# rageworx/libsrcnn

Hardware: AMD Instinct MI355X
Metric: megapixels/sec SRCNN Y-channel (2x upscale) (higher is better)
Workload: dtype f32

## Files before the change

libsrcnn_amd/build.py:

```python
import os
import subprocess
import sys

HERE = os.path.dirname(os.path.abspath(__file__))
CSRC = os.path.join(HERE, "csrc")
LIBDIR = os.path.join(HERE, "lib")
LIB = os.path.join(LIBDIR, "libsrcnn_amd.so")

SOURCES = ["srcnn_kernels.hip", "srcnn_fused_f16.hip", "srcnn_yuv_planes.hip", "srcnn_yuv_packed.hip", "srcnn_rgb.hip", "srcnn_rgb_window.hip", "srcnn_yuv_window.hip", "srcnn_yuv_packed_window.hip", "srcnn_window.hip", "srcnn_rect_list.hip", "srcnn_rgb_rect_list.hip", "srcnn_rect_list_call.cpp", "srcnn_rgb_rect_list_call.cpp", "srcnn_capi.cpp", "srcnn_frames.cpp", "srcnn_pipeline.cpp", "srcnn_comm.cpp", "dropin.cpp"]
DEPS = SOURCES + ["../../tools/srcnntest.cpp", "../../tools/srcnnyuv.cpp", "srcnn_kernels.h", "srcnn_yuv.h", "srcnn_rgb.h", "srcnn_window.h", "srcnn_frame_rules.h", "srcnn_frame_args.hpp", "srcnn_rect_source.hpp", "srcnn_rect_atlas.hpp", "srcnn_rgb_rect_atlas.hpp", "srcnn_rect_list.h", "srcnn_pixel_io.h", "srcnn_colour_rules.h", "srcnn_window_tile.h", "srcnn_yuv_packed_fields.h", "srcnn_host.hpp", "srcnn_owned.hpp", "srcnn_settings.hpp", "srcnn_watchdog.hpp", "resample_table.hpp", "srcnn_weights.inc",
                  "../../include/srcnn_amd.h", "../../include/srcnn_amd_debug.h", "../../include/srcnn_amd_yuv.h", "../../include/srcnn_amd_yuv_ex.h", "../../include/srcnn_amd_yuv_packed.h", "../../include/srcnn_amd_rgb.h", "../../include/srcnn_amd_rect.h", "../../include/srcnn_amd_rect_list.h", "../../include/srcnn_amd_rgb_rect.h", "../../include/srcnn_amd_rgb_rect_list.h", "../../include/srcnn_amd_yuv_rect.h", "../../include/srcnn_amd_yuv_packed_rect.h",
                  "../../include/libsrcnn_dropin.h", "exports.map"]

FLAGS = ["--offload-arch=gfx950", "-O3", "-ffp-contract=off", "-fPIC", "-std=c++17",
         "-fvisibility=hidden", "-Wall", "-Wno-unused-result", "-Wno-unused-value", "-Wno-ignored-attributes", "-D__HIP_PLATFORM_AMD__"]


EXTRA_FLAGS = {"srcnn_fused_f16.hip": ["-fno-slp-vectorize"] + os.environ.get("SRCNN_FUSED_CFLAGS", "").split()}


def hipcc():
    for c in (os.environ.get("HIPCC"), "/opt/rocm/bin/hipcc", "hipcc"):
        if c and (os.path.isabs(c) and os.path.exists(c) or not os.path.isabs(c)):
            return c
# ... 18 lines not shown
def stale():
    if not all(os.path.exists(p) for p in (LIB, STAMP, os.path.join(LIBDIR, "libsrcnn.so"), os.path.join(LIBDIR, "libsrcnn.a"))):
        return True
    try:
        return open(STAMP).read().strip() != source_digest()
    except OSError:
        return True


def _region(src, start_pat, end_pat):
    import re
    m = re.search(start_pat, src)
    if not m:
        return None
    e = re.search(end_pat, src[m.end():])
    return src[m.start():m.end() + (e.start() if e else len(src) - m.end())]


def kernel_source_sha(name="k_conv12_mfma"):
    import hashlib
    import re
    src = open(os.path.join(CSRC, "srcnn_kernels.hip")).read()
    m = re.search(r"template <[^>]*>\s*__global__[^\n]*void %s\(" % re.escape(name), src)
    if not m and name == "k_conv3_sparse":
        m = re.search(r"// =+\n// conv3, strict, skipping all-zero channel windows", src)
        if m and not re.search(r"__global__[^\n]*void k_conv3_sparse\(", src[m.end():src.find("// ====", src.find("__global__", m.end()))]):
            m = None
    if not m:
        return None
    end = src.find("// ====", src.find("__global__", m.end()) if name == "k_conv3_sparse" else m.end())
    parts = [src[m.start():end if end > 0 else len(src)]]
    extra = []
    if name == "k_conv12_mfma":
        extra = [_region(src, r"constexpr int M_NW\b", r"\n// One tap-step"),
                 _region(src, r"__device__ __forceinline__ void rs_dma_dword\(", r"\n}\n"),
                 _region(src, r"void conv12_grid_info\(", r"\n}\n"),
                 _region(src, r"void launch_conv12_mfma\(", r"\n}\n"),
                 _region(open(os.path.join(CSRC, "srcnn_capi.cpp")).read(), r"void run_conv12\(", r"\n}\n")]
    elif name == "k_conv3":
        extra = [_region(src, r"constexpr int C3_TW\b", r"\ntemplate <bool STRICT"),
                 _region(src, r"__device__ __forceinline__ void rs_dma_dword\(", r"\n}\n"),
                 _region(src, r"void launch_conv3\(", r"\n}\n")]
    elif name == "k_conv3_sparse":
        extra = [_region(src, r"constexpr int C3_TW\b", r"\ntemplate <bool STRICT"),
                 _region(src, r"__device__ __forceinline__ void rs_dma_dword\(", r"\n}\n"),
                 _region(src, r"void launch_layer3\(", r"\n}\n"),
                 _region(src, r"void launch_conv3\(", r"\n}\n")]
    if any(e is None for e in extra):
        return None
    h = hashlib.sha256()
    for part in parts + extra:
        h.update(part.encode())
        h.update(b"\0")
    return h.hexdigest()


STRICT_DIR = os.path.join(LIBDIR, "strict")
STRICT_LIB = os.path.join(STRICT_DIR, "libsrcnn_amd.so")


def build_strict_only(force=False, verbose=True):
# ... 76 lines not shown
```

libsrcnn_amd/csrc/srcnn_capi.cpp:

```cpp
#include <dlfcn.h>
#include <hip/hip_runtime.h>
#include <sys/prctl.h>
#include <sys/syscall.h>
#include <unistd.h>

#include <algorithm>
#include <cstdio>
#include <cstdlib>
#include <cstring>
#include <string>
#include <thread>

#include "resample_table.hpp"
#include <chrono>
#include <sys/auxv.h>
#include <unistd.h>

#include "../../include/srcnn_amd_rect.h"
#include "srcnn_frame_args.hpp"
#include "srcnn_host.hpp"
#include "srcnn_rect_source.hpp"
#include "srcnn_window.h"

namespace srcnn {
// ... 674 lines not shown
{
    unsigned long long* clk = nullptr;
    if (G.clock_probe.load(std::memory_order_relaxed) && c.cx->clock_buf)
        clk = c.cx->clock_buf + 2 * (size_t)(c.cx->clock_n.fetch_add(1) % kClockSlots);
    unsigned* queue = nullptr;
    hipStreamCaptureStatus cap = hipStreamCaptureStatusNone;
    const bool foreign_capture = c.s && c.ws && !c.ws->frozen && hipStreamIsCapturing(c.s, &cap) == hipSuccess && cap == hipStreamCaptureStatusActive;
    if (foreign_capture) clk = nullptr;
    if (c.ws && settings().conv12_queue && !foreign_capture) {
        if (c.ws->queue && c.ws->queue_dirty) {
            if (hipMemsetAsync(c.ws->queue, 0, 2 * sizeof(unsigned), c.s) == hipSuccess) c.ws->queue_dirty = false;
            else (void)hipGetLastError();
        }
        if (!c.ws->queue && !c.ws->frozen) {
            void* q = nullptr;
            if (hipMalloc(&q, 2 * sizeof(unsigned)) == hipSuccess && hipMemsetAsync(q, 0, 2 * sizeof(unsigned), c.s) == hipSuccess) c.ws->queue = static_cast<unsigned*>(q);
            else { (void)hipFree(q); (void)hipGetLastError(); }
        }
        queue = c.ws->queue;
    }
    launch_conv12_mfma(Y, W, H, y_row_base, y_rows, C2, plane, row0, rows, c.relax(), c.cx->num_cus, c.s, clk, queue);
}

DevAxisTable view_of(const TableRef& t) { return t->view(); }

int resample_src_rows(Call& c, const YSource& src, unsigned sw, unsigned sh, unsigned dw, unsigned dh, int filter,
                      unsigned r0, unsigned r1, float* d_dst)
{
    Workspace& ws = *c.ws;
    hipStream_t s = c.s;
    const float* d_in = src.plane;
    if (sw == dw && sh == dh) {
        if (!d_in) return fail(SRCNN_E_UNSUPPORTED, "identity-size resample needs a float plane");
        HIP_TRY(hipMemcpyAsync(d_dst, d_in + (size_t)r0 * sw, sizeof(float) * (size_t)(r1 - r0) * sw,
                               hipMemcpyDeviceToDevice, s));
        return SRCNN_OK;
    }
    TableRef tv, th;
    int rc;
    if (dw > sw && sh != dh) {
        if ((rc = get_table(c, filter, dw, sw, th))) return rc;
        if ((rc = get_table(c, filter, dh, sh, tv))) return rc;
        if (!settings().resample_2pass &&
            launch_rs2d(src, sw, sh, d_dst, dw, dh, r0, r1 - r0, view_of(tv), view_of(th), s)) return SRCNN_OK;
    }
    if (!d_in) return fail(SRCNN_E_UNSUPPORTED, "this resample shape needs a float source plane");
// ... 107 lines not shown
    if (fused) {
        {
            StageTimer t(SRCNN_STAGE_RESAMPLE, c);
            if ((rc = resample_src_rows(c, src, w, h, dw, dh, filter, ua, ub, ws.up.data()))) return rc;
        }
        {
            StageTimer t(SRCNN_STAGE_CONV12, c);
            launch_fused_f16(ws.up.data(), (int)dw, (int)dh, (int)ua, (int)(ub - ua), d_out, (int)r0, (int)(r1 - r0), cx.fused_w.data(),
                             cx.num_cus, c.s);
        }
        HIP_TRY(hipGetLastError());
        return SRCNN_OK;
    }
#endif
    if ((rc = ws.grow(ws.c2, (size_t)C2N * dw * (cb - ca)))) return rc;
    TraceRange tr("srcnn y_path rows [%u,%u) of %ux%u", r0, r1, dw, dh);
    {
        StageTimer t(SRCNN_STAGE_RESAMPLE, c);
        if ((rc = resample_src_rows(c, src, w, h, dw, dh, filter, ua, ub, ws.up.data()))) return rc;
    }
    const size_t plane = (size_t)dw * (cb - ca);
    {
        StageTimer t(SRCNN_STAGE_CONV12, c);
        run_conv12(c, ws.up.data(), (int)dw, (int)dh, (int)ua, (int)(ub - ua), ws.c2.data(), plane, (int)ca, (int)(cb - ca));
    }
    {
        StageTimer t(SRCNN_STAGE_CONV3, c);
        launch_layer3(ws.c2.data(), plane, (int)dw, (int)dh, (int)ca, (int)(cb - ca), d_out, (int)r0, (int)(r1 - r0),
                     c.relax(), c.s);
    }
    if (const hipError_t e = hipGetLastError(); e != hipSuccess) {
        ws.queue_dirty = true;
        return fail(SRCNN_E_HIP, "y_path_rows: %s", hipGetErrorString(e));
    }
    return SRCNN_OK;
}

int y_path_source_rows(Call& c, unsigned h, unsigned dh, int filter, unsigned r0, unsigned r1, unsigned& lo, unsigned& hi)
{
    const unsigned ca = r0 >= 2 ? r0 - 2 : 0, cb = std::min(dh, r1 + 2);
    const unsigned ua = ca >= 4 ? ca - 4 : 0, ub = std::min(dh, cb + 4);
    if (h == dh) { lo = ua; hi = ub; return SRCNN_OK; }
    TableRef tv;
    int rc = get_table(c, filter, dh, h, tv);
    if (rc) return rc;
    tv->source_span(ua, ub, lo, hi);
    hi = std::min(hi, h);
// ... 85 lines not shown
        {
            StageTimer t(SRCNN_STAGE_RESAMPLE, c);
            if ((rc = resample_window(c, d_in, in_stride, in_x0, in_y0, w, h, dw, dh, filter, uax, ubx, ua, ub, ws.up.data()))) return rc;
        }
        {
            StageTimer t(SRCNN_STAGE_CONV12, c);
            launch_fused_f16(ws.up.data(), (int)Ww, (int)dh, (int)ua, (int)(ub - ua), ws.win.data(), (int)r0, (int)(r1 - r0), cx.fused_w.data(),
                             cx.num_cus, c.s);
        }
        launch_window_copy(interior, Ww, d_out, out_stride, (int)(x1 - x0), (int)(r1 - r0), c.s);
        HIP_TRY(hipGetLastError());
        return SRCNN_OK;
    }
#endif
    if ((rc = ws.grow(ws.c2, (size_t)C2N * Ww * (cb - ca)))) return rc;
    TraceRange tr("srcnn y_path rect [%u,%u)x[%u,%u) of %ux%u", x0, x1, r0, r1, dw, dh);
    {
        StageTimer t(SRCNN_STAGE_RESAMPLE, c);
        if ((rc = resample_window(c, d_in, in_stride, in_x0, in_y0, w, h, dw, dh, filter, uax, ubx, ua, ub, ws.up.data()))) return rc;
    }
    const size_t plane = (size_t)Ww * (cb - ca);
    {
        StageTimer t(SRCNN_STAGE_CONV12, c);
        run_conv12(c, ws.up.data(), (int)Ww, (int)dh, (int)ua, (int)(ub - ua), ws.c2.data(), plane, (int)ca, (int)(cb - ca));
    }
    {
        StageTimer t(SRCNN_STAGE_CONV3, c);
        launch_layer3(ws.c2.data(), plane, (int)Ww, (int)dh, (int)ca, (int)(cb - ca), ws.win.data(), (int)r0, (int)(r1 - r0), c.relax(), c.s);
    }
    launch_window_copy(interior, Ww, d_out, out_stride, (int)(x1 - x0), (int)(r1 - r0), c.s);
    if (const hipError_t e = hipGetLastError(); e != hipSuccess) {
        ws.queue_dirty = true;
        return fail(SRCNN_E_HIP, "y_path_rect: %s", hipGetErrorString(e));
    }
    return SRCNN_OK;
}

}

int y_path_rect(Call& c, const float* d_in, size_t in_stride, unsigned in_x0, unsigned in_y0, unsigned w, unsigned h, unsigned dw,
                unsigned dh, int filter, unsigned x0, unsigned y0, unsigned x1, unsigned y1, float* d_out, size_t out_stride, bool whole_plane)
{
    if (x1 > dw || x0 >= x1 || y1 > dh || y0 >= y1) return fail(SRCNN_E_ARG, "rect [%u,%u)x[%u,%u) outside %ux%u", x0, x1, y0, y1, dw, dh);
    if (dh > (1u << 20) || h > (1u << 20) || dw > 0x7fffffu || (y1 - y0) > 65535u * 16u)
        return fail(SRCNN_E_UNSUPPORTED, "output %ux%u too large", dw, dh);
    if (x0 == 0 && x1 == dw && whole_plane && in_x0 == 0 && in_y0 == 0 && in_stride == w && out_stride == dw)
        return y_path_range(c, d_in, w, h, dw, dh, filter, y0, y1, d_out);
// ... 421 lines not shown

extern "C++" {
namespace srcnn {

int check_rect_geometry(unsigned w, unsigned h, unsigned dw, unsigned dh, int filter, unsigned x0, unsigned y0, unsigned rw, unsigned rh)
{
    if (w == 0 || h == 0 || rw == 0 || rh == 0) return fail(SRCNN_E_ARG, "zero dimension (%ux%u, rect %ux%u)", w, h, rw, rh);
    if (dw == 0 || dh == 0) return fail(SRCNN_E_SCALE, "scaled size %ux%u", dw, dh);
    if (filter < 0 || filter > 4) return fail(SRCNN_E_ARG, "bad filter %d", filter);
    if ((unsigned long long)x0 + rw > dw || (unsigned long long)y0 + rh > dh)
        return fail(SRCNN_E_ARG, "rect %ux%u at (%u,%u) is not inside the %ux%u output", rw, rh, x0, y0, dw, dh);
    return SRCNN_OK;
}

int check_rect_limits(unsigned w, unsigned h, unsigned dw, unsigned dh, unsigned rh)
{
    if (h > (1u << 20) || dh > (1u << 20) || dw > 0x7fffffu || rh > 65535u * 16u || (unsigned long long)w * h > 0x7fffffffULL)
        return fail(SRCNN_E_UNSUPPORTED, "%ux%u -> %ux%u is beyond the Y path's limits", w, h, dw, dh);
    return SRCNN_OK;
}

void run_layers12(const Call& c, const float* Y, int W, int H, int y_row_base, int y_rows, float* C2, size_t plane, int row0, int rows)
{
    run_conv12(c, Y, W, H, y_row_base, y_rows, C2, plane, row0, rows);
}

}
}

int srcnn_rect_abi_version(void) { return SRCNN_AMD_RECT_VERSION; }

int srcnn_y_path_rect_source(unsigned w, unsigned h, unsigned dw, unsigned dh, int filter, unsigned x0, unsigned y0, unsigned rw,
                             unsigned rh, unsigned* sx0, unsigned* sy0, unsigned* sw, unsigned* sh)
{
    int rc;
    if ((rc = check_rect_geometry(w, h, dw, dh, filter, x0, y0, rw, rh))) return rc;
    if ((rc = check_rect_limits(w, h, dw, dh, rh))) return rc;
    unsigned lx, hx, ly, hy;
    y_path_rect_source_span(w, h, dw, dh, filter, x0, y0, x0 + rw, y0 + rh, lx, hx, ly, hy);
    if (sx0) *sx0 = lx;
    if (sy0) *sy0 = ly;
    if (sw) *sw = hx - lx;
    if (sh) *sh = hy - ly;
    return SRCNN_OK;
}

int srcnn_y_path_rect_f32_dev(const float* d_in, size_t in_pitch, unsigned w, unsigned h, unsigned dw, unsigned dh, int filter,
// ... 135 lines not shown

int srcnn_conv3_f32_dev(const float* d_c2, unsigned w, unsigned h, float* d_out, void* stream)
{
    int rc;
    if ((rc = check_plane(d_c2, w, h, d_out))) return rc;
    if (h > 65535u * 16u) return fail(SRCNN_E_UNSUPPORTED, "too many rows");
    if (!ctx_for_stream(stream)) return SRCNN_E_NODEVICE;
    Call c;
    c.mode = G.mode.load();
    launch_layer3(d_c2, (size_t)w * h, (int)w, (int)h, 0, (int)h, d_out, 0, (int)h, c.relax(), (hipStream_t)stream);
    HIP_TRY(hipGetLastError());
    return SRCNN_OK;
}

int srcnn_conv12_f32_dev(const float* d_y, unsigned w, unsigned h, float* d_c2, void* stream)
{
    int rc;
    if ((rc = check_plane(d_y, w, h, d_c2))) return rc;
    if (h > 65535u * 4u) return fail(SRCNN_E_UNSUPPORTED, "too many rows");
    Call c;
    c.cx = ctx_for_stream(stream);
    if (!c.cx) return SRCNN_E_NODEVICE;
    c.s = (hipStream_t)stream; c.mode = G.mode.load();
    run_conv12(c, d_y, (int)w, (int)h, 0, (int)h, d_c2, (size_t)w * h, 0, (int)h);
    HIP_TRY(hipGetLastError());
    return SRCNN_OK;
}

int srcnn_axis_table(int filter, unsigned dst_len, unsigned src_len, int* left, int* right, double* weights)
{
    if (dst_len == 0 || src_len == 0) return fail(SRCNN_E_ARG, "zero length");
    const srcnn::AxisTable t = srcnn::build_axis_table(filter, dst_len, src_len);
    if (left) memcpy(left, t.first.data(), sizeof(int) * dst_len);
    if (right) memcpy(right, t.last.data(), sizeof(int) * dst_len);
    if (weights) memcpy(weights, t.weight.data(), sizeof(double) * t.weight.size());
    return t.window;
}

int srcnn_fused_diag(const float* d_up, unsigned w, unsigned h, float* d_out, unsigned long long* d_dbg, void* stream)
{
    int rc;
    if ((rc = check_plane(d_up, w, h, d_out))) return rc;
#ifdef SRCNN_STRICT_ONLY
    (void)d_dbg; (void)stream;
    return fail(SRCNN_E_UNSUPPORTED, "strict-only build: the fused fp16 kernel is not compiled in");
#else
    Ctx* cx = ctx_for_stream(stream);
// ... 30 lines not shown
```

libsrcnn_amd/csrc/srcnn_kernels.h:

```cpp
#pragma once
#include <hip/hip_runtime.h>
#include <stddef.h>

namespace srcnn {

constexpr int C1N = 64;
constexpr int C2N = 32;
enum : int {
    RELAX_L1 = 1,
    RELAX_L2 = 2,
    RELAX_L3_X64 = 4,
    RELAX_L3_F32 = 8,
    RELAX_FAST = RELAX_L1 | RELAX_L2 | RELAX_L3_F32
};
constexpr int kWeightCount = 64 + 64 * 81 + 32 + 32 * 64 + 1 + 32 * 25;

struct DevWeights {
    float w1t[81][C1N];
    float b1[C1N];
    float w2[C2N][C1N];
    float b2[C2N];
    float w3[C2N][25];
    float b3;
    float pad_[3];
// ... 35 lines not shown
    float pad_[3];
};

hipError_t upload_weights(const DevWeights& w);
hipError_t fused_f16_prepare();
void launch_fused_f16(const float* Y, int W, int H, int y_row_base, int y_rows, float* out, int out_row0, int out_rows,
                      const FusedF16Weights* d_blob, int num_cus, hipStream_t s, unsigned long long* dbg = nullptr);

void launch_resample_cols(const float* src, int w, int src_row_base, float* dst, int dst_row0, int dst_rows,
                          const DevAxisTable& t, hipStream_t s);
void launch_resample_rows(const float* src, int src_w, float* dst, int dst_w, int rows, const DevAxisTable& t,
                          hipStream_t s);
bool launch_rs2d(const YSource& src, int src_w, int src_h, float* dst, int dst_w, int dst_h, int dst_row0, int dst_rows,
                 const DevAxisTable& tv, const DevAxisTable& th, hipStream_t s);
hipError_t rs2d_prepare();
bool rs2d_fits(int np, int src_w, int src_h, int dst_w, int dst_h, int r0, int r1, const DevAxisTable& tv, const DevAxisTable& th);
bool launch_merge_fused(const unsigned char* rgb_src, int src_w, int src_h, int depth, const float* Yp,
                        unsigned char* rgb_out, unsigned char* conv_opt, int dst_w, int dst_h, int dst_row0, int dst_rows,
                        const DevAxisTable& tv, const DevAxisTable& th, hipStream_t s);
hipError_t conv12_mfma_prepare();
void launch_conv12_mfma(const float* Y, int W, int H, int y_row_base, int y_rows, float* C2, size_t plane_stride, int out_row0,
                        int out_rows, int relax, int num_cus, hipStream_t s, unsigned long long* clk = nullptr,
                        unsigned* queue = nullptr);
void conv12_grid_info(int num_cus, int* blocks, int* tile_rows);
constexpr int kConv12TileRows = 16, kConv12BlocksPerCU = 2;
void launch_conv3(const float* C2, size_t plane_stride, int W, int H, int c2_row_base, int c2_rows, float* out,
                  int out_row0, int out_rows, int relax, hipStream_t s);
void launch_layer3(const float* C2, size_t plane_stride, int W, int H, int c2_row_base, int c2_rows, float* out,
                   int out_row0, int out_rows, int relax, hipStream_t s);
void launch_conv1_planes(const float* Y, int W, int H, float* C1, hipStream_t s);
void launch_conv2_planes(const float* C1, size_t n, float* C2v, hipStream_t s);
void launch_rgb_split(const unsigned char* rgb, size_t n, int d, float* Yp, float* Cb, float* Cr, float* A,
                      hipStream_t s);
void launch_ycc_merge(const float* Yp, const float* Cb, const float* Cr, const float* A, size_t n, int d,
                      unsigned char* rgb, unsigned char* conv_opt, hipStream_t s);

}
```

libsrcnn_amd/csrc/srcnn_kernels.hip:

```cpp
#include <hip/hip_runtime.h>
#include <type_traits>
#include <stdint.h>
#include <stdlib.h>
#include <algorithm>
#include "srcnn_kernels.h"
#include "srcnn_settings.hpp"

#pragma clang fp contract(off)

namespace srcnn {

__constant__ DevWeights cW;

hipError_t upload_weights(const DevWeights& w)
{
    return hipMemcpyToSymbol(HIP_SYMBOL(cW), &w, sizeof(DevWeights));
}

__device__ __forceinline__ int clampi(int v, int lo, int hi) { return v < lo ? lo : (v > hi ? hi : v); }

__global__ __launch_bounds__(256) void k_resample_cols(
    const float* __restrict__ src, int w, int src_row_base,
    float* __restrict__ dst, int dst_row0, int dst_rows,
    const int* __restrict__ first, const int* __restrict__ taps, const double* __restrict__ wt, int stride)
// ... 707 lines not shown
                float* dst = C2 + (size_t)(row - out_row0) * W + x + (size_t)(4 * half) * plane_stride;
#pragma unroll
                for (int r = 0; r < 16; ++r) {
                    const int m = 8 * (r >> 2) + (r & 3);
                    dst[(size_t)m * plane_stride] = fmaxf(acc2[r] + B2s[half * 16 + r], 0.f);
                }
            }
        }
        if (dyn && tid == 0) qslot[(it + 1) & 1] = drawn;
        item = next_item;
    }
    if (dyn && tid == 0) {
        if (atomicAdd(queue + 1, 1u) == gridDim.x - 1) { queue[0] = 0u; queue[1] = 0u; }
    }
    if (clk && blockIdx.x == 0) {
        __syncthreads();
        if (threadIdx.x == 0) {
            clk[0] = __builtin_amdgcn_s_memtime() - clk_c0;
            clk[1] = __builtin_amdgcn_s_memrealtime() - clk_r0;
        }
    }
}

constexpr int C3_TW = 64, C3_TH = 16;
constexpr int C3_LW = C3_TW + 4, C3_LH = C3_TH + 4;
constexpr int C3_CH = C3_LH * C3_LW;
static_assert(C3_LH % 4 == 0, "row slots");
constexpr int c3_mc(bool sdma) { return sdma ? 2 : 4; }

template <bool STRICT, bool OFF64 = false, bool X64 = false, bool SDMA = false>
__global__ __launch_bounds__(256, SDMA ? 6 : 3) void k_conv3(
    const float* __restrict__ C2, size_t plane_stride, int W, int H, int c2_row_base, int c2_rows,
    float* __restrict__ out, int out_row0, int out_rows, int weights_by_dma)
{
    constexpr int C3_MC = c3_mc(SDMA);
    constexpr int C3_BODY = C3_MC * C3_LH / 4;
    constexpr int C3_HALO = (C3_MC * C3_LH * 4 + 255) / 256;
    __shared__ float tile[2][C3_MC * C3_CH];
    __shared__ __attribute__((aligned(16))) float w3s[X64 ? C2N * 50 : C2N * 30];

    const int tx0 = blockIdx.x * C3_TW;
    const int ty0 = out_row0 + blockIdx.y * C3_TH;
    const int tid = threadIdx.x, lane = tid & 63, wv = tid >> 6;
    const int c2_last = c2_row_base + c2_rows - 1;
    if constexpr (X64) {
        double* w3d = reinterpret_cast<double*>(w3s);
// ... 676 lines not shown
    a.yp = Yp; a.out_rgb = rgb_out; a.out_conv = conv_opt;
    a.dst_w = dst_w; a.dst_row0 = dst_row0; a.dst_rows = dst_rows;
    a.sr = p.sr; a.tpb = p.tpb;
    a.vfirst = tv.first; a.vtaps = tv.taps; a.vwt = tv.weight; a.vstride = tv.stride;
    a.hfirst = th.first; a.htaps = th.taps; a.hwt = th.weight; a.hstride = th.stride;
    a.vec = (dst_w % 4 == 0) && aligned_to(Yp, 16) && aligned_to(rgb_out, 4) && (!conv_opt || aligned_to(conv_opt, 4));
    if (depth == 3) { if (conv_opt) rs2d_dispatch<2, 3, true>(p, a, s); else rs2d_dispatch<2, 3, false>(p, a, s); }
    else            { if (conv_opt) rs2d_dispatch<2, 4, true>(p, a, s); else rs2d_dispatch<2, 4, false>(p, a, s); }
    return true;
}

template <int RELAX, bool LD>
static hipError_t prep_one()
{
    return hipFuncSetAttribute(reinterpret_cast<const void*>(&k_conv12_mfma<RELAX, LD>),
                               hipFuncAttributeMaxDynamicSharedMemorySize, (int)(sizeof(float) * m_lds_floats(LD)));
}

hipError_t conv12_mfma_prepare()
{
    hipError_t e;
    if ((e = prep_one<0, true>()) != hipSuccess) return e;
    if ((e = prep_one<0, false>()) != hipSuccess) return e;
#ifndef SRCNN_STRICT_ONLY
    if ((e = prep_one<1, true>()) != hipSuccess) return e;
    if ((e = prep_one<2, true>()) != hipSuccess) return e;
    if ((e = prep_one<3, true>()) != hipSuccess) return e;
#endif
    return hipSuccess;
}

void conv12_grid_info(int num_cus, int* blocks, int* tile_rows)
{
    if (blocks) *blocks = M_BPC * num_cus;
    if (tile_rows) *tile_rows = M_TH;
}

void launch_conv12_mfma(const float* Y, int W, int H, int y_row_base, int y_rows, float* C2, size_t plane_stride, int out_row0,
                        int out_rows, int relax, int num_cus, hipStream_t s, unsigned long long* clk, unsigned* queue)
{
    if (out_rows <= 0) return;
    const int prune = settings().conv12_prune ? 1 : 0;
    const int tiles_x = (int)cdiv(W, M_TW), tiles_y = (int)cdiv(out_rows, M_TH);
    const int ntiles = tiles_x * tiles_y;
    const int cap = M_BPC * num_cus;
    const int grid = ntiles >= cap ? cap : (settings().conv12_spread ? std::min(4 * ntiles, cap) : ntiles);
#define CONV12_GO(R, LD) hipLaunchKernelGGL((k_conv12_mfma<R, LD>), dim3(grid), dim3(64 * M_NW), sizeof(float) * m_lds_floats(LD), s, Y, W, H, \
                                           y_row_base, y_rows, C2, plane_stride, out_row0, out_rows, tiles_x, ntiles, clk, LD ? queue : nullptr, prune)
#ifdef SRCNN_STRICT_ONLY
    (void)relax;
    if (settings().conv12_dma) CONV12_GO(0, true); else CONV12_GO(0, false);
#else
    switch (relax & 3) {
    case 0: if (settings().conv12_dma) CONV12_GO(0, true); else CONV12_GO(0, false); break;
    case 1: CONV12_GO(1, true); break;
    case 2: CONV12_GO(2, true); break;
    default: CONV12_GO(3, true); break;
    }
#endif
#undef CONV12_GO
}

void launch_conv3(const float* C2, size_t plane_stride, int W, int H, int c2_row_base, int c2_rows, float* out,
                  int out_row0, int out_rows, int relax, hipStream_t s)
{
    if (out_rows <= 0) return;
#ifndef SRCNN_STRICT_ONLY
    const bool strict = !(relax & (RELAX_L3_X64 | RELAX_L3_F32));
    const bool wide_planes = (size_t)c2_rows * (size_t)W * sizeof(float) >= ((size_t)1 << 32);
    if (relax & RELAX_L3_X64) {
        const dim3 gx(cdiv(W, 64), cdiv(out_rows, 16));
        if (wide_planes)
            hipLaunchKernelGGL((k_conv3<true, true, true>), gx, dim3(256), 0, s, C2, plane_stride, W, H, c2_row_base, c2_rows, out, out_row0, out_rows, 0);
        else
            hipLaunchKernelGGL((k_conv3<true, false, true>), gx, dim3(256), 0, s, C2, plane_stride, W, H, c2_row_base, c2_rows, out, out_row0, out_rows, 0);
        return;
    }
    if (!strict) {
        dim3 gridf(cdiv(W, CF_TW), cdiv(out_rows, CF_TH));
        hipLaunchKernelGGL(k_conv3_fast, gridf, dim3(256), 0, s, C2, plane_stride, W, H, c2_row_base, c2_rows, out,
                           out_row0, out_rows);
        return;
    }
#else
    (void)relax;
// ... 165 lines not shown
```

libsrcnn_amd/csrc/srcnn_settings.hpp:

```cpp
#pragma once
#include <cstddef>
#include <string>

#define SRCNN_SETTINGS(X)                                                                                                          \
                                                                                                            \
    X(S, devices,          "SRCNN_DEVICES",          "",    "unset = device 0, `all`, `0,1,...`", "contexts of a process that never calls `srcnn_init*` (an id may repeat: virtual contexts on one device)") \
    X(I, max_workspace_mb, "SRCNN_MAX_WORKSPACE_MB", 4608, "MiB (API twin `srcnn_set_workspace_limit`)", "layer-2 scratch one pass may hold; larger ranges are banded, bit-identically.  The default holds a whole 7680x4320 output frame (4.25 GB); lower it where memory is short: 2048 costs -1...+2 % by box, 512 +2 %, 256 +9 % (`profiles/r06_lowmem.txt`); 16384 until round 6") \
    X(I, max_lanes,        "SRCNN_MAX_LANES",        4,     "1...64", "concurrent `ProcessSRCNN` calls per context before callers queue") \
    X(B, numa,             "SRCNN_NUMA",             1,     "0/1", "place page-locked staging on the device's NUMA node (the caller's memory policy is saved and restored)") \
    X(I, comm_timeout_ms,  "SRCNN_COMM_TIMEOUT_MS",  60000, "ms, 0 = none (API twin `srcnn_comm_set_timeout_ms`)", "deadline of every wait on a peer") \
    X(B, comm_check,       "SRCNN_COMM_CHECK",       1,     "0/1", "all-reduce a checksum of every new gather table across the ranks before the first gather that uses it") \
    X(S, rccl_lib,         "SRCNN_RCCL_LIB",         "",    "path", "load this RCCL instead of the one next to the bound `libamdhip64` (site builds; the test-suite's one-device stand-in).  A trust boundary: the named file's code runs in the process; refused under secure execution (`AT_SECURE`)") \
    X(I, async_chain,      "SRCNN_ASYNC_CHAIN",      1,     "0/1/2", "order the kernels of consecutive asynchronous `ProcessSRCNN` jobs: 0 = not at all, 1 = on the host, 2 = with device-side event waits") \
    X(B, trace,            "SRCNN_TRACE",            0,     "0/1", "one stderr line per `srcnn_process_u8` share (setup / bands / stamps)") \
    X(B, roctx,            "SRCNN_ROCTX",            0,     "0/1", "roctx ranges for `rocprofv3 --marker-trace`") \
    X(S, bands,            "SRCNN_BANDS",            "",    "`f0,f1,...`", "band fractions of a large `ProcessSRCNN` image instead of the planned cuts") \
    X(I, graph_max_cpu_pct, "SRCNN_GRAPH_MAX_CPU_PCT", 10,  "0...100, 0 = never fall back", "`srcnn_y_upscale2x_f32_stream(use_graph = 1)`: hipGraph replay is kept only while the process's CPU time per replayed frame stays below this share of the frame's wall time (plain launches cost 6-8 % of a 4K frame; replay on ROCm 7.2 costs 20 % in a fresh process and ~100 % -- a runtime thread spinning from launch to completion -- in a process with more streams); above it the stream goes on with plain launches: same kernels, same overlap") \
    X(B, prefault,         "SRCNN_PREFAULT",         1,     "0/1", "pre-fault the fresh result pages of `ProcessSRCNN` in the background") \
    X(I, prefault_threads, "SRCNN_PREFAULT_THREADS", 1,     ">= 1", "helpers of that pre-faulting") \
    X(B, thp,              "SRCNN_THP",              1,     "0/1", "huge-page hint on large result blocks") \
    X(B, spin_wait,        "SRCNN_SPIN_WAIT",        0,     "0/1", "host waits through the runtime (holds a core) instead of polling") \
    X(B, device_wait_in,   "SRCNN_DEVICE_WAIT_IN",   0,     "0/1", "bands wait for their stage-in device-side (a runtime thread stays busy)") \
                   \
    X(B, conv12_queue,     "SRCNN_CONV12_QUEUE",     1,     "0/1", "layer 1+2: tiles drawn from a global counter vs dealt with a static stride") \
    X(B, conv12_dma,       "SRCNN_CONV12_DMA",       1,     "0/1", "layer 1+2: weights and Y tiles staged by LDS-DMA one tile ahead vs load, wait, `ds_write`") \
    X(B, conv12_prune,     "SRCNN_CONV12_PRUNE",     1,     "0/1", "layer 1+2: strict layer 2 skips the 15 near-dead layer-1 channels in every 32-pixel segment where they are all zero vs always multiplies all 64") \
    X(B, conv12_spread,    "SRCNN_CONV12_SPREAD",    1,     "0/1", "layer 1+2: small launches dealt in quarter tiles over up to 4x more workgroups") \
    X(B, conv3_wdma,       "SRCNN_CONV3_WDMA",       1,     "0/1", "layer 3: packed weight image staged by LDS-DMA vs a plain loop") \
    X(B, conv3_off64,      "SRCNN_CONV3_OFF64",      0,     "0/1", "layer 3: 64-bit plane offsets (chosen automatically for planes of 4 GiB or more)") \
    X(B, conv3_skip,       "SRCNN_CONV3_SKIP",       1,     "0/1", "layer 3: `k_conv3_sparse`, where a wave skips a layer-2 channel of the candidate set {1, 13, 26, 29} whose activations it has just read as all zero over its 68x8 window, vs `k_conv3`, which always runs all 32") \
    X(B, rs_dma,           "SRCNN_RS_DMA",           1,     "0/1", "resampler: `k_rs2d_dma` (source patch by LDS-DMA) vs `k_rs2d` for plane sources") \
    X(I, rs_tpb,           "SRCNN_RS_TPB",           0,     "0 = auto, 1...16", "resampler: row tiles a block marches through") \
    X(B, resample_2pass,   "SRCNN_RESAMPLE_2PASS",   0,     "0/1", "resampler: always the two generic passes (`k_resample_cols/rows`, what down-scales use); implies the unfused colour shell") \
    X(B, shell_unfused,    "SRCNN_SHELL_UNFUSED",    0,     "0/1", "colour shell as split + plane resamples + merge instead of fused into the resampler") \
    X(B, rgb_rect_unfused, "SRCNN_RGB_RECT_UNFUSED", 0,     "0/1", "RGB(A) rect call: window unpack + window plane resamples + pack for every shape instead of `k_rgb_window_merge` for up-scales") \
    X(B, yuv_rect_unfused, "SRCNN_YUV_RECT_UNFUSED", 0,     "0/1", "YUV rect call: chroma by window unpack + window plane resamples + pack for every shape instead of `k_yuv_window_chroma` for up-scales") \
    X(B, yuv_packed_rect_unfused, "SRCNN_YUV_PACKED_RECT_UNFUSED", 0, "0/1", "packed YUV rect call: window unpack + window plane resamples + pack for every shape instead of `k_yuvp_window_merge` for up-scales") \
    X(B, rect_list_unfused, "SRCNN_RECT_LIST_UNFUSED", 0,   "0/1", "rect list call: every item as a single rect call instead of the windows of small rects packed into one atlas per layer launch") \
    X(I, rect_list_single_samples, "SRCNN_RECT_LIST_SINGLE_SAMPLES", 2097152, "samples of a cell, (rw + 12) x (rh + 12)", "rect list call: items whose cell has at least this many samples run as single rect calls.  Started at 524288 (512 tiles of 64x16, one round of the persistent layer-1+2 grid); the sweep of `profiles/rect_list_probe.txt` found no crossover there -- 16 rects of 768x768 and 1024x1024 were still 1.4x and 1.3x faster batched than looped -- so it stands at 2^21, the largest cell that sweep measures.  The RGB(A) rect list call routes by the same threshold") \
    X(B, rgb_rect_list_unfused, "SRCNN_RGB_RECT_LIST_UNFUSED", 0, "0/1", "RGB(A) rect list call: every item as a single RGB(A) rect call instead of small rects sharing one atlas per layer launch, with Y read and colour merged by `k_rgb_list_resample` / `k_rgb_list_merge`")

namespace srcnn {

struct Settings {
#define SRCNN_SET_B(m, d) bool m = (d) != 0;
#define SRCNN_SET_I(m, d) long m = (d);
#define SRCNN_SET_S(m, d) std::string m = d;
#define X(kind, member, env, def, values, effect) SRCNN_SET_##kind(member, def)
    SRCNN_SETTINGS(X)
// ... 12 lines not shown
```

Baseline: 3766.

## Add tiered zero-skipping conv12 kernel that prunes often-zero layer-1 channels

Adds k_conv12_tiers, a variant of the fused layer 1+2 MFMA kernel. Per 32-pixel segment it ballots whether the near-dead channels, and separately a second set of often-zero layer-1 channels, are all zero after ReLU. It then runs a reduced layer-2 MFMA loop over only the live channels of that tier. It is enabled by default through a new setting and routed via run_layer12, aiming to cut layer-2 MFMA work on inputs with sparse activations, at the cost of extra ballots, branches and code size.

```diff
diff --git a/libsrcnn_amd/build.py b/libsrcnn_amd/build.py
--- a/libsrcnn_amd/build.py
+++ b/libsrcnn_amd/build.py
@@ -64,13 +64,15 @@
     import re
     src = open(os.path.join(CSRC, "srcnn_kernels.hip")).read()
     m = re.search(r"template <[^>]*>\s*__global__[^\n]*void %s\(" % re.escape(name), src)
-    if not m and name == "k_conv3_sparse":
-        m = re.search(r"// =+\n// conv3, strict, skipping all-zero channel windows", src)
-        if m and not re.search(r"__global__[^\n]*void k_conv3_sparse\(", src[m.end():src.find("// ====", src.find("__global__", m.end()))]):
+    banners = {"k_conv3_sparse": r"// =+\n// conv3, strict, skipping all-zero channel windows",
+               "k_conv12_tiers": r"// =+\n// conv12, strict, nested zero tiers in layer 2"}
+    if not m and name in banners:
+        m = re.search(banners[name], src)
+        if m and not re.search(r"__global__[^\n]*void %s\(" % name, src[m.end():src.find("// ====", src.find("__global__", m.end()))]):
             m = None
     if not m:
         return None
-    end = src.find("// ====", src.find("__global__", m.end()) if name == "k_conv3_sparse" else m.end())
+    end = src.find("// ====", src.find("__global__", m.end()) if name in banners else m.end())
     parts = [src[m.start():end if end > 0 else len(src)]]
     extra = []
     if name == "k_conv12_mfma":
@@ -79,6 +81,14 @@
                  _region(src, r"void conv12_grid_info\(", r"\n}\n"),
                  _region(src, r"void launch_conv12_mfma\(", r"\n}\n"),
                  _region(open(os.path.join(CSRC, "srcnn_capi.cpp")).read(), r"void run_conv12\(", r"\n}\n")]
+    elif name == "k_conv12_tiers":
+        capi = open(os.path.join(CSRC, "srcnn_capi.cpp")).read()
+        extra = [_region(src, r"constexpr int M_NW\b", r"\n// One tap-step"),
+                 _region(src, r"__device__ __forceinline__ void rs_dma_dword\(", r"\n}\n"),
+                 _region(src, r"void launch_conv12_tiers\(", r"\n}\n"),
+                 _region(src, r"void conv12_grid_info\(", r"\n}\n"),
+                 _region(capi, r"void run_layer12\(", r"\n}\n"),
+                 _region(capi, r"void run_conv12\(", r"\n}\n")]
     elif name == "k_conv3":
         extra = [_region(src, r"constexpr int C3_TW\b", r"\ntemplate <bool STRICT"),
                  _region(src, r"__device__ __forceinline__ void rs_dma_dword\(", r"\n}\n"),
diff --git a/libsrcnn_amd/csrc/srcnn_capi.cpp b/libsrcnn_amd/csrc/srcnn_capi.cpp
--- a/libsrcnn_amd/csrc/srcnn_capi.cpp
+++ b/libsrcnn_amd/csrc/srcnn_capi.cpp
@@ -720,6 +720,35 @@
     launch_conv12_mfma(Y, W, H, y_row_base, y_rows, C2, plane, row0, rows, c.relax(), c.cx->num_cus, c.s, clk, queue);
 }
 
+void run_layer12(const Call& c, const float* Y, int W, int H, int y_row_base, int y_rows, float* C2, size_t plane, int row0,
+                 int rows)
+{
+    if (c.relax() != 0 || !settings().conv12_dma || !settings().conv12_prune || !settings().conv12_tiers) {
+        run_conv12(c, Y, W, H, y_row_base, y_rows, C2, plane, row0, rows);
+        return;
+    }
+    unsigned long long* clk = nullptr;
+    if (G.clock_probe.load(std::memory_order_relaxed) && c.cx->clock_buf)
+        clk = c.cx->clock_buf + 2 * (size_t)(c.cx->clock_n.fetch_add(1) % kClockSlots);
+    unsigned* queue = nullptr;
+    hipStreamCaptureStatus cap = hipStreamCaptureStatusNone;
+    const bool foreign_capture = c.s && c.ws && !c.ws->frozen && hipStreamIsCapturing(c.s, &cap) == hipSuccess && cap == hipStreamCaptureStatusActive;
+    if (foreign_capture) clk = nullptr;
+    if (c.ws && settings().conv12_queue && !foreign_capture) {
+        if (c.ws->queue && c.ws->queue_dirty) {
+            if (hipMemsetAsync(c.ws->queue, 0, 2 * sizeof(unsigned), c.s) == hipSuccess) c.ws->queue_dirty = false;
+            else (void)hipGetLastError();
+        }
+        if (!c.ws->queue && !c.ws->frozen) {
+            void* q = nullptr;
+            if (hipMalloc(&q, 2 * sizeof(unsigned)) == hipSuccess && hipMemsetAsync(q, 0, 2 * sizeof(unsigned), c.s) == hipSuccess) c.ws->queue = static_cast<unsigned*>(q);
+            else { (void)hipFree(q); (void)hipGetLastError(); }
+        }
+        queue = c.ws->queue;
+    }
+    launch_conv12_tiers(Y, W, H, y_row_base, y_rows, C2, plane, row0, rows, c.cx->num_cus, c.s, clk, queue);
+}
+
 DevAxisTable view_of(const TableRef& t) { return t->view(); }
 
 int resample_src_rows(Call& c, const YSource& src, unsigned sw, unsigned sh, unsigned dw, unsigned dh, int filter,
@@ -873,7 +902,7 @@
     const size_t plane = (size_t)dw * (cb - ca);
     {
         StageTimer t(SRCNN_STAGE_CONV12, c);
-        run_conv12(c, ws.up.data(), (int)dw, (int)dh, (int)ua, (int)(ub - ua), ws.c2.data(), plane, (int)ca, (int)(cb - ca));
+        run_layer12(c, ws.up.data(), (int)dw, (int)dh, (int)ua, (int)(ub - ua), ws.c2.data(), plane, (int)ca, (int)(cb - ca));
     }
     {
         StageTimer t(SRCNN_STAGE_CONV3, c);
@@ -1005,7 +1034,7 @@
     const size_t plane = (size_t)Ww * (cb - ca);
     {
         StageTimer t(SRCNN_STAGE_CONV12, c);
-        run_conv12(c, ws.up.data(), (int)Ww, (int)dh, (int)ua, (int)(ub - ua), ws.c2.data(), plane, (int)ca, (int)(cb - ca));
+        run_layer12(c, ws.up.data(), (int)Ww, (int)dh, (int)ua, (int)(ub - ua), ws.c2.data(), plane, (int)ca, (int)(cb - ca));
     }
     {
         StageTimer t(SRCNN_STAGE_CONV3, c);
@@ -1473,7 +1502,7 @@
 
 void run_layers12(const Call& c, const float* Y, int W, int H, int y_row_base, int y_rows, float* C2, size_t plane, int row0, int rows)
 {
-    run_conv12(c, Y, W, H, y_row_base, y_rows, C2, plane, row0, rows);
+    run_layer12(c, Y, W, H, y_row_base, y_rows, C2, plane, row0, rows);
 }
 
 }
@@ -1655,7 +1684,7 @@
     c.cx = ctx_for_stream(stream);
     if (!c.cx) return SRCNN_E_NODEVICE;
     c.s = (hipStream_t)stream; c.mode = G.mode.load();
-    run_conv12(c, d_y, (int)w, (int)h, 0, (int)h, d_c2, (size_t)w * h, 0, (int)h);
+    run_layer12(c, d_y, (int)w, (int)h, 0, (int)h, d_c2, (size_t)w * h, 0, (int)h);
     HIP_TRY(hipGetLastError());
     return SRCNN_OK;
 }
diff --git a/libsrcnn_amd/csrc/srcnn_kernels.h b/libsrcnn_amd/csrc/srcnn_kernels.h
--- a/libsrcnn_amd/csrc/srcnn_kernels.h
+++ b/libsrcnn_amd/csrc/srcnn_kernels.h
@@ -81,6 +81,8 @@
 void launch_conv12_mfma(const float* Y, int W, int H, int y_row_base, int y_rows, float* C2, size_t plane_stride, int out_row0,
                         int out_rows, int relax, int num_cus, hipStream_t s, unsigned long long* clk = nullptr,
                         unsigned* queue = nullptr);
+void launch_conv12_tiers(const float* Y, int W, int H, int y_row_base, int y_rows, float* C2, size_t plane_stride, int out_row0,
+                         int out_rows, int num_cus, hipStream_t s, unsigned long long* clk = nullptr, unsigned* queue = nullptr);
 void conv12_grid_info(int num_cus, int* blocks, int* tile_rows);
 constexpr int kConv12TileRows = 16, kConv12BlocksPerCU = 2;
 void launch_conv3(const float* C2, size_t plane_stride, int W, int H, int c2_row_base, int c2_rows, float* out,
diff --git a/libsrcnn_amd/csrc/srcnn_kernels.hip b/libsrcnn_amd/csrc/srcnn_kernels.hip
--- a/libsrcnn_amd/csrc/srcnn_kernels.hip
+++ b/libsrcnn_amd/csrc/srcnn_kernels.hip
@@ -753,6 +753,247 @@
     }
 }
 
+constexpr int MT_TIERS = 2;
+constexpr unsigned long long MT_TIER[MT_TIERS] = {
+    M_DEAD,
+    0x40174e0a77e5640aull,
+};
+constexpr bool mt_nested()
+{
+    for (int t = 1; t < MT_TIERS; ++t)
+        if ((MT_TIER[t] & MT_TIER[t - 1]) != MT_TIER[t - 1] || MT_TIER[t] == MT_TIER[t - 1]) return false;
+    return MT_TIER[0] == M_DEAD;
+}
+static_assert(mt_nested(), "every tier contains the tier below, and the first is M_DEAD");
+template <unsigned long long MASK>
+constexpr unsigned long long mt_lanes(int blk, int r)
+{
+    const int f = 32 * blk + 8 * (r >> 2) + (r & 3);
+    return ((MASK >> f) & 1 ? 0x00000000ffffffffull : 0ull) | ((MASK >> (f + 4)) & 1 ? 0xffffffff00000000ull : 0ull);
+}
+template <unsigned long long MASK>
+constexpr int mt_live_count(int blk)
+{
+    int n = 0;
+    for (int f = 0; f < 32; ++f) n += !((MASK >> (32 * blk + f)) & 1);
+    return n;
+}
+template <unsigned long long MASK>
+constexpr int mt_live_nth(int blk, int n)
+{
+    for (int f = 0; f < 32; ++f)
+        if (!((MASK >> (32 * blk + f)) & 1) && n-- == 0) return f;
+    return -1;
+}
+static_assert(mt_live_count<MT_TIER[MT_TIERS - 1]>(0) >= 4 && mt_live_count<MT_TIER[MT_TIERS - 1]>(1) >= 4, "two pairs per block are fetched ahead");
+
+__global__ __launch_bounds__(64 * M_NW, 4) void k_conv12_tiers(
+    const float* __restrict__ Y, int W, int H, int y_row_base, int y_rows,
+    float* __restrict__ C2, size_t plane_stride, int out_row0, int out_rows, int tiles_x, int ntiles,
+    unsigned long long* __restrict__ clk, unsigned* __restrict__ queue)
+{
+    constexpr int NW = M_NW, NT = 64 * NW, TH = M_TH, YT = M_YT;
+    unsigned long long clk_c0 = 0, clk_r0 = 0;
+    if (clk && blockIdx.x == 0) { clk_c0 = __builtin_amdgcn_s_memtime(); clk_r0 = __builtin_amdgcn_s_memrealtime(); }
+    extern __shared__ __attribute__((aligned(16))) float lds[];
+    float* W1s = lds;
+    float* W2s = W1s + M_W1;
+    float* B1s = W2s + M_W2;
+    float* B2s = B1s + M_B1;
+    float* Yt  = B2s + M_B2;
+    float* C1s = Yt + m_ybufs(true) * YT;
+
+    const int tid = threadIdx.x, lane = tid & 63, wv = tid >> 6, half = lane >> 5, col = lane & 31;
+
+    const int wave_e0w = __builtin_amdgcn_readfirstlane(tid & ~63);
+#pragma unroll
+    for (int i = 0; i < (M_W1 + NT - 1) / NT; ++i) {
+        const int e = tid + i * NT;
+        if (e < M_W1) rs_dma_dword(&cW.w1t[0][0] + e, W1s + i * NT + wave_e0w);
+    }
+#pragma unroll
+    for (int i = 0; i < (M_W2 + NT - 1) / NT; ++i) {
+        const int e = tid + i * NT;
+        if (e < M_W2) { const int fp = e >> 6, l = e & 63; rs_dma_dword(&cW.w2[l & 31][2 * fp + (l >> 5)], W2s + i * NT + wave_e0w); }
+    }
+    if (tid < 64) {
+        const int hf = tid >> 5, r = tid & 31;
+        rs_dma_dword(&cW.b1[32 * (r >> 4) + 8 * ((r & 15) >> 2) + 4 * hf + (r & 3)], B1s);
+    }
+    if (tid < 32) {
+        const int hf = tid >> 4, r = tid & 15;
+        rs_dma_dword(&cW.b2[8 * (r >> 2) + 4 * hf + (r & 3)], B2s);
+    }
+    float* myC1 = C1s + wv * M_C1;
+    const f32x32 zero32 = {};
+
+    const int full = (ntiles / (int)gridDim.x) * (int)gridDim.x;
+    const int nitems = full + 4 * (ntiles - full);
+    constexpr int NPRE = (YT + NT - 1) / NT;
+    auto tile_of = [&](int item, int& s0, int& s1) {
+        int tile = item; s0 = 0; s1 = 4;
+        if (item >= full) { const int i = item - full; tile = full + (i >> 2); s0 = i & 3; s1 = s0 + 1; }
+        return tile;
+    };
+    const int wave_e0 = wave_e0w;
+    auto request = [&](int item, float* buf) {
+        int q0, q1;
+        const int tile = tile_of(item, q0, q1);
+        const int tyi = tile / tiles_x, txi = tile - tyi * tiles_x;
+        const int tx0 = txi * M_TW, ty0 = out_row0 + tyi * TH;
+#pragma unroll
+        for (int i = 0; i < NPRE; ++i) {
+            const int e = tid + i * NT;
+            if (e < YT) {
+                const int r = e / M_LW, c = e - r * M_LW;
+                const int gy = clampi(clampi(ty0 + r - 4, 0, H - 1), y_row_base, y_row_base + y_rows - 1), gx = clampi(tx0 + c - 4, 0, W - 1);
+                rs_dma_dword(Y + (size_t)(gy - y_row_base) * W + gx, buf + i * NT + wave_e0);
+            }
+        }
+    };
+    int* qslot = reinterpret_cast<int*>(C1s + NW * M_C1);
+    const bool dyn = queue != nullptr;
+    int it = 0;
+    int item = blockIdx.x;
+    if (item < nitems) request(item, Yt);
+    if (dyn && tid == 0 && item < nitems) qslot[0] = (int)gridDim.x + (int)atomicAdd(queue, 1u);
+    for (; item < nitems; ++it) {
+        int s0, s1;
+        const int tile = tile_of(item, s0, s1);
+        const int tyi = tile / tiles_x, txi = tile - tyi * tiles_x;
+        const int tx0 = txi * M_TW, ty0 = out_row0 + tyi * TH;
+        int next_item = item + (int)gridDim.x;
+        int drawn = 0x7fffffff;
+        const float* Ytc = Yt + (it & 1) * YT;
+        asm volatile("s_waitcnt vmcnt(0)" ::: "memory");
+        __syncthreads();
+        if (dyn) next_item = __builtin_amdgcn_readfirstlane(qslot[it & 1]);
+        if (next_item < nitems) request(next_item, Yt + ((it + 1) & 1) * YT);
+        if (dyn && tid == 0 && next_item < nitems) drawn = (int)gridDim.x + (int)atomicAdd(queue, 1u);
+
+#pragma unroll 1
+        for (int s = s0; s < s1; ++s) {
+            const int sg = wv * 4 + s;
+            const int trow = sg >> 1, seg = sg & 1;
+            const float* yrow = Ytc + trow * M_LW + seg * 32 + col;
+
+            f32x32 acc = zero32;
+            {
+                float a1 = W1s[lane], b1 = yrow[0];
+                float a2 = W1s[64 + lane], b2 = yrow[1];
+#pragma unroll
+                for (int t = 0; t < 81; ++t) {
+                    f32x32 d = __builtin_amdgcn_mfma_f32_32x32x1f32(a1, b1, zero32, 0, 0, 0);
+                    PIN(d);
+                    a1 = a2; b1 = b2;
+                    if (t + 2 < 81) {
+                        a2 = W1s[(t + 2) * 64 + lane];
+                        b2 = yrow[((t + 2) / 9) * M_LW + ((t + 2) % 9)];
+                    }
+                    if (t == 0) acc = d; else acc += d;
+                    PIN(acc);
+                    __builtin_amdgcn_sched_barrier(0);
+                }
+            }
+            f32x16 acc2 = {};
+#pragma unroll
+            for (int blk = 0; blk < 2; ++blk) {
+                constexpr unsigned long long D1 = MT_TIER[0], D2 = MT_TIER[MT_TIERS - 1] & ~MT_TIER[0];
+                constexpr unsigned long long LO = 0x00000000ffffffffull, HI = 0xffffffff00000000ull;
+                unsigned any1 = 0, lo1 = 0, hi1 = 0, any2 = 0, lo2 = 0, hi2 = 0;
+#pragma unroll
+                for (int r = 0; r < 16; ++r) {
+                    const float v = fmaxf(acc[16 * blk + r] + B1s[half * 32 + 16 * blk + r], 0.f);
+                    const int f = 8 * (r >> 2) + (r & 3);
+                    myC1[(f + 4 * half) * 32 + col] = v;
+                    const unsigned u = __float_as_uint(v);
+                    if (mt_lanes<D1>(blk, r) == (LO | HI)) any1 |= u; else if (mt_lanes<D1>(blk, r) == LO) lo1 |= u; else if (mt_lanes<D1>(blk, r) == HI) hi1 |= u;
+                    if (mt_lanes<D2>(blk, r) == (LO | HI)) any2 |= u; else if (mt_lanes<D2>(blk, r) == LO) lo2 |= u; else if (mt_lanes<D2>(blk, r) == HI) hi2 |= u;
+                }
+                const bool live1 = __builtin_amdgcn_ballot_w64(((any1 | (half ? hi1 : lo1)) & 0x7fffffffu) != 0u) != 0;
+                const bool live2 = __builtin_amdgcn_ballot_w64(((any2 | (half ? hi2 : lo2)) & 0x7fffffffu) != 0u) != 0;
+                __builtin_amdgcn_fence(__ATOMIC_RELEASE, "wavefront");
+                __builtin_amdgcn_wave_barrier();
+                __builtin_amdgcn_fence(__ATOMIC_ACQUIRE, "wavefront");
+
+                const float* w2p = W2s + blk * 16 * 64;
+                float a1 = w2p[lane], b1 = myC1[lane];
+                float a2 = w2p[64 + lane], b2 = myC1[64 + lane];
+                auto tier_body = [&](auto BLK, auto T) {
+                    constexpr int B = decltype(BLK)::value;
+                    constexpr unsigned long long MASK = MT_TIER[decltype(T)::value];
+                    constexpr int NL = mt_live_count<MASK>(B), NP = (NL + 1) / 2;
+                    auto off = [&](auto P) {
+                        constexpr int p = decltype(P)::value, fa = mt_live_nth<MASK>(B, 2 * p), fb = 2 * p + 1 < NL ? mt_live_nth<MASK>(B, 2 * p + 1) : fa;
+                        return lane + 32 * fa + (lane & 32) * (fb - fa - 1);
+                    };
+                    const int o0 = off(std::integral_constant<int, 0>{}), o1 = off(std::integral_constant<int, 1>{});
+                    a1 = w2p[o0]; b1 = myC1[o0];
+                    a2 = w2p[o1]; b2 = myC1[o1];
+                    m_static_for<NP>([&](auto P) {
+                        constexpr int p = decltype(P)::value;
+                        f32x32 d = __builtin_amdgcn_mfma_f32_32x32x1f32(a1, b1, zero32, 0, 0, 0);
+                        PIN(d);
+                        a1 = a2; b1 = b2;
+                        if constexpr (p + 2 < NP) { const int o = off(std::integral_constant<int, p + 2>{}); a2 = w2p[o]; b2 = myC1[o]; }
+                        if constexpr (B == 0 && p == 0) acc2 = __builtin_shufflevector(d, d, 0, 1, 2, 3, 4, 5, 6, 7, 8, 9, 10, 11, 12, 13, 14, 15);
+                        else
+                        acc2 += __builtin_shufflevector(d, d, 0, 1, 2, 3, 4, 5, 6, 7, 8, 9, 10, 11, 12, 13, 14, 15);
+                        if constexpr (2 * p + 1 < NL)
+                        acc2 += __builtin_shufflevector(d, d, 16, 17, 18, 19, 20, 21, 22, 23, 24, 25, 26, 27, 28, 29, 30, 31);
+                        PIN(acc2);
+                        __builtin_amdgcn_sched_barrier(0);
+                    });
+                };
+                const std::integral_constant<int, 0> B0{};
+                const std::integral_constant<int, 1> B1{};
+                if (!live1 && !live2) {
+                    if (blk == 0) tier_body(B0, std::integral_constant<int, 1>{}); else tier_body(B1, std::integral_constant<int, 1>{});
+                } else if (!live1) {
+                    if (blk == 0) tier_body(B0, std::integral_constant<int, 0>{}); else tier_body(B1, std::integral_constant<int, 0>{});
+                } else {
+#pragma unroll
+                    for (int fp = 0; fp < 16; ++fp) {
+                        f32x32 d = __builtin_amdgcn_mfma_f32_32x32x1f32(a1, b1, zero32, 0, 0, 0);
+                        PIN(d);
+                        a1 = a2; b1 = b2;
+                        if (fp + 2 < 16) { a2 = w2p[(fp + 2) * 64 + lane]; b2 = myC1[(fp + 2) * 64 + lane]; }
+                        if (blk == 0 && fp == 0) acc2 = __builtin_shufflevector(d, d, 0, 1, 2, 3, 4, 5, 6, 7, 8, 9, 10, 11, 12, 13, 14, 15);
+                        else
+                        acc2 += __builtin_shufflevector(d, d, 0, 1, 2, 3, 4, 5, 6, 7, 8, 9, 10, 11, 12, 13, 14, 15);
+                        acc2 += __builtin_shufflevector(d, d, 16, 17, 18, 19, 20, 21, 22, 23, 24, 25, 26, 27, 28, 29, 30, 31);
+                        PIN(acc2);
+                        __builtin_amdgcn_sched_barrier(0);
+                    }
+                }
+                __builtin_amdgcn_wave_barrier();
+            }
+
+            const int row = ty0 + trow, x = tx0 + seg * 32 + col;
+            if (row < out_row0 + out_rows && row < H && x < W) {
+                float* dst = C2 + (size_t)(row - out_row0) * W + x + (size_t)(4 * half) * plane_stride;
+#pragma unroll
+                for (int r = 0; r < 16; ++r) {
+                    const int m = 8 * (r >> 2) + (r & 3);
+                    dst[(size_t)m * plane_stride] = fmaxf(acc2[r] + B2s[half * 16 + r], 0.f);
+                }
+            }
+        }
+        if (dyn && tid == 0) qslot[(it + 1) & 1] = drawn;
+        item = next_item;
+    }
+    if (dyn && tid == 0) {
+        if (atomicAdd(queue + 1, 1u) == gridDim.x - 1) { queue[0] = 0u; queue[1] = 0u; }
+    }
+    if (clk && blockIdx.x == 0) {
+        __syncthreads();
+        if (threadIdx.x == 0) {
+            clk[0] = __builtin_amdgcn_s_memtime() - clk_c0;
+            clk[1] = __builtin_amdgcn_s_memrealtime() - clk_r0;
+        }
+    }
+}
+
 constexpr int C3_TW = 64, C3_TH = 16;
 constexpr int C3_LW = C3_TW + 4, C3_LH = C3_TH + 4;
 constexpr int C3_CH = C3_LH * C3_LW;
@@ -1475,6 +1716,8 @@
     hipError_t e;
     if ((e = prep_one<0, true>()) != hipSuccess) return e;
     if ((e = prep_one<0, false>()) != hipSuccess) return e;
+    if ((e = hipFuncSetAttribute(reinterpret_cast<const void*>(&k_conv12_tiers), hipFuncAttributeMaxDynamicSharedMemorySize,
+                                 (int)(sizeof(float) * m_lds_floats(true)))) != hipSuccess) return e;
 #ifndef SRCNN_STRICT_ONLY
     if ((e = prep_one<1, true>()) != hipSuccess) return e;
     if ((e = prep_one<2, true>()) != hipSuccess) return e;
@@ -1514,6 +1757,19 @@
 #undef CONV12_GO
 }
 
+void launch_conv12_tiers(const float* Y, int W, int H, int y_row_base, int y_rows, float* C2, size_t plane_stride, int out_row0,
+                         int out_rows, int num_cus, hipStream_t s, unsigned long long* clk, unsigned* queue)
+{
+    if (out_rows <= 0) return;
+    const int tiles_x = (int)cdiv(W, M_TW), tiles_y = (int)cdiv(out_rows, M_TH);
+    const int ntiles = tiles_x * tiles_y;
+    int cap = 0;
+    conv12_grid_info(num_cus, &cap, nullptr);
+    const int grid = ntiles >= cap ? cap : (settings().conv12_spread ? std::min(4 * ntiles, cap) : ntiles);
+    hipLaunchKernelGGL(k_conv12_tiers, dim3(grid), dim3(64 * M_NW), sizeof(float) * m_lds_floats(true), s, Y, W, H, y_row_base, y_rows,
+                       C2, plane_stride, out_row0, out_rows, tiles_x, ntiles, clk, queue);
+}
+
 void launch_conv3(const float* C2, size_t plane_stride, int W, int H, int c2_row_base, int c2_rows, float* out,
                   int out_row0, int out_rows, int relax, hipStream_t s)
 {
diff --git a/libsrcnn_amd/csrc/srcnn_settings.hpp b/libsrcnn_amd/csrc/srcnn_settings.hpp
--- a/libsrcnn_amd/csrc/srcnn_settings.hpp
+++ b/libsrcnn_amd/csrc/srcnn_settings.hpp
@@ -25,6 +25,7 @@
     X(B, conv12_queue,     "SRCNN_CONV12_QUEUE",     1,     "0/1", "layer 1+2: tiles drawn from a global counter vs dealt with a static stride") \
     X(B, conv12_dma,       "SRCNN_CONV12_DMA",       1,     "0/1", "layer 1+2: weights and Y tiles staged by LDS-DMA one tile ahead vs load, wait, `ds_write`") \
     X(B, conv12_prune,     "SRCNN_CONV12_PRUNE",     1,     "0/1", "layer 1+2: strict layer 2 skips the 15 near-dead layer-1 channels in every 32-pixel segment where they are all zero vs always multiplies all 64") \
+    X(B, conv12_tiers,     "SRCNN_CONV12_TIERS",     1,     "0/1", "layer 1+2: `k_conv12_tiers`, where strict layer 2 also skips the often-zero layer-1 channels {1, 3, 10, 13, 14, 16, 29} / {33, 48, 49, 52, 62} of a 32-channel block in every 32-pixel segment where they and the block's near-dead channels are all zero, vs `k_conv12_mfma`, which skips the near-dead channels only (needs `SRCNN_CONV12_DMA` and `SRCNN_CONV12_PRUNE`)") \
     X(B, conv12_spread,    "SRCNN_CONV12_SPREAD",    1,     "0/1", "layer 1+2: small launches dealt in quarter tiles over up to 4x more workgroups") \
     X(B, conv3_wdma,       "SRCNN_CONV3_WDMA",       1,     "0/1", "layer 3: packed weight image staged by LDS-DMA vs a plain loop") \
     X(B, conv3_off64,      "SRCNN_CONV3_OFF64",      0,     "0/1", "layer 3: 64-bit plane offsets (chosen automatically for planes of 4 GiB or more)") \
```

Measured after the change: 3810 (median of 6 runs). +1.2%, better.
